# Huangying-Zhan/DF-VO

Hardware: AMD Instinct MI355X
Metric: KITTI-odom frames/sec (DF-VO per-pair tracking hot path: monodepth2 + LiteFlowNet fwd/bwd + kp selection + E/H RANSAC + scale) (higher is better)
Workload: dtype f32 (f16x3 split products: two f16 planes per operand = 22 mantissa bits, three exact products per term, fp32 accumulate; direct one- / two-channel heads exact fp32)

## Files before the change

df-vo_amd/csrc/conv_taps_f16s.hip:

```cpp
#include "dfvo_common.h"


namespace dfvo {

#include "conv_epi.h"
#include "conv_f16_split.h"

typedef unsigned int u32x4t __attribute__((ext_vector_type(4)));
typedef unsigned int u32x2t __attribute__((ext_vector_type(2)));
typedef __attribute__((address_space(4))) const u32x4t cu32x4t;

template <int TH, int TC, int NP = 3, int PF = 3>
__global__ __launch_bounds__(64 * TH) void conv_taps_f16s_kernel(const ConvParams p, int G, int pxd, int wcols, int wrows) {
    extern __shared__ __attribute__((aligned(16))) unsigned char taps_lds[];
    constexpr int NT = 64 * TH;
    const int t = threadIdx.x, lane = t & 63;
    const int wave = __builtin_amdgcn_readfirstlane(t >> 6);
    const int lp = lane & 31, kb = lane >> 5;
    const int tiles_x = (p.Wo + 31) / 32, tiles_y = (p.Ho + TH - 1) / TH;
    const int nb = gridDim.x;
    int bid = blockIdx.x;
    {
        const int q = nb >> 3, r = nb & 7, xcd = bid & 7, k = bid >> 3;
        bid = (xcd < r ? xcd * (q + 1) : r * (q + 1) + (xcd - r) * q) + k;
    }
    const int n = bid / (tiles_y * tiles_x);
    const int trem = bid - n * (tiles_y * tiles_x);
    const int oy0 = (trem / tiles_x) * TH, ox0 = (trem % tiles_x) * 32;
    const int iy0 = oy0 * p.stride - p.pad_h, ix0 = ox0 * p.stride - p.pad_w;

    float amax = 0.f;
    const int npix = wrows * wcols;
    const int zoff = npix * pxd;
    if (t < 4) reinterpret_cast<unsigned*>(taps_lds + zoff)[t] = 0u;
    {
        const int dpx = NT / G, dcg = NT - dpx * G;
        const int dwy = dpx / wcols, dwx = dpx - dwy * wcols;
        int px = t / G, cg = t - px * G;
        int wy = px / wcols, wx = px - wy * wcols;
        constexpr int LB = 4;
        const int nitems = npix * G;
        for (int it = t; it < nitems; it += NT * LB) {
            f32x4 xb[LB];
            int pxb[LB], cgb[LB];
#pragma unroll
            for (int u = 0; u < LB; ++u) {
                const bool live = it + u * NT < nitems;
                const int iy = iy0 + wy, ix = ix0 + wx;
                const bool v = live && iy >= 0 && iy < p.H && ix >= 0 && ix < p.W;
                pxb[u] = live ? px : -1;
                cgb[u] = cg;
                xb[u] = f32x4{0.f, 0.f, 0.f, 0.f};
                if (v) xb[u] = *reinterpret_cast<const f32x4*>(p.src0 + ((size_t)(n * p.H + iy) * p.W + ix) * p.cs0 + p.co0 + cg * 4);
                cg += dcg;
                int cpx = dpx;
                if (cg >= G) {
                    cg -= G;
                    cpx += 1;
                }
                px += cpx;
                wx += dwx + (cpx - dpx);
                wy += dwy;
                if (wx >= wcols) {
                    wx -= wcols;
                    wy += 1;
                }
                if (wx >= wcols) {
                    wx -= wcols;
                    wy += 1;
                }
            }
#pragma unroll
            for (int u = 0; u < LB; ++u) {
                if (pxb[u] < 0) continue;
                h16x4 hi, lo;
                unsigned char* d = taps_lds + (size_t)pxb[u] * pxd + cgb[u] * 8;
                if constexpr (NP == 3) {
                    split_f16_planes(xb[u], &hi, &lo, amax);
                    *reinterpret_cast<h16x4*>(d) = hi;
                    *reinterpret_cast<h16x4*>(d + G * 8) = lo;
                } else {
                    split_f16_hi(xb[u], &hi, amax);
                    *reinterpret_cast<h16x4*>(d) = hi;
                }
            }
        }
    }
    const int S = p.f16g_steps;
    const int rowb = wcols * pxd, lo_off = G * 8;
    int* const otab = reinterpret_cast<int*>(taps_lds + zoff + 16);
    for (int i = t; i < S * 4; i += NT) {
        const unsigned e = p.f16g_tab[i];
        const int ky = e & 31, kx = (e >> 5) & 31, cg = (int)(e >> 16) >> 2;
        otab[i] = ((e >> 10) & 1u) ? ky * rowb + kx * pxd + cg * 8 : -1;
    }
    __syncthreads();

    const unsigned short* const wbase = p.wf16g + (size_t)(kb * 32 + lp) * 8;
    const size_t w_step_stride = (size_t)p.wf16g_cout_pad * 32;
    const int lane_base = (wave * p.stride * wcols + lp * p.stride) * pxd;

    h16x8 rw[PF][TC][2];
    u32x2t rx[PF][2][2];
    int nl = 0;
    u32x2t oo = *reinterpret_cast<const u32x2t*>(otab + 2 * kb);
    auto load_step = [&](int st) {
        const int o0 = (int)oo[0], o1 = (int)oo[1];
        oo = *reinterpret_cast<const u32x2t*>(otab + (nl + 1 < S ? nl + 1 : S - 1) * 4 + 2 * kb);
#pragma unroll
        for (int j = 0; j < 2; ++j) {
            const int o = j ? o1 : o0;
            const int a_hi = o < 0 ? zoff : lane_base + o;
            const int a_lo = o < 0 ? zoff + 8 : lane_base + o + lo_off;
            rx[st][j][0] = *reinterpret_cast<const u32x2t*>(taps_lds + a_hi);
            if constexpr (NP == 3) rx[st][j][1] = *reinterpret_cast<const u32x2t*>(taps_lds + a_lo);
        }
        const unsigned short* g = wbase + (size_t)nl * w_step_stride;
#pragma unroll
        for (int i = 0; i < TC; ++i) {
            rw[st][i][0] = *reinterpret_cast<const h16x8*>(g + (size_t)i * 1024);
            if constexpr (NP == 3) rw[st][i][1] = *reinterpret_cast<const h16x8*>(g + (size_t)i * 1024 + 512);
        }
        ++nl;
    };
    f32x16 am[TC], ax[TC];
#pragma unroll
    for (int i = 0; i < TC; ++i)
#pragma unroll
        for (int e = 0; e < 16; ++e) am[i][e] = ax[i][e] = 0.f;
#pragma unroll
    for (int d = 0; d < PF; ++d)
        if (d < S) load_step(d);
    for (int s = 0; s < S; s += PF) {
#pragma unroll
        for (int u = 0; u < PF; ++u) {
            if (s + u < S) {
                const u32x4t hq = {rx[u][0][0][0], rx[u][0][0][1], rx[u][1][0][0], rx[u][1][0][1]};
                u32x4t lq = {0u, 0u, 0u, 0u};
                if constexpr (NP == 3) lq = u32x4t{rx[u][0][1][0], rx[u][0][1][1], rx[u][1][1][0], rx[u][1][1][1]};
                const h16x8 xh = __builtin_bit_cast(h16x8, hq), xl = __builtin_bit_cast(h16x8, lq);
                h16x8 wh[TC], wl[TC];
#pragma unroll
                for (int i = 0; i < TC; ++i) {
                    wh[i] = rw[u][i][0];
                    if constexpr (NP == 3) wl[i] = rw[u][i][1];
                }
                if (s + u + PF < S) load_step(u);
                if constexpr (NP == 3) {
#pragma unroll
                    for (int i = 0; i < TC; ++i) ax[i] = __builtin_amdgcn_mfma_f32_32x32x16_f16(wh[i], xl, ax[i], 0, 0, 0);
#pragma unroll
                    for (int i = 0; i < TC; ++i) ax[i] = __builtin_amdgcn_mfma_f32_32x32x16_f16(wl[i], xh, ax[i], 0, 0, 0);
                }
#pragma unroll
                for (int i = 0; i < TC; ++i) am[i] = __builtin_amdgcn_mfma_f32_32x32x16_f16(wh[i], xh, am[i], 0, 0, 0);
            }
        }
    }
    if (amax > F16S_MAX) atomicAdd(p.f16s_clamp_ctr, 1u);

    const int oy = oy0 + wave, ox = ox0 + lp;
    if (oy >= p.Ho || ox >= p.Wo) return;
    float* const drow = p.dst + (((size_t)n * p.Ho + oy) * p.Wo + ox) * p.dst_cs + p.dst_co;
    const float slope = p.act == ACT_LEAKY ? p.act_param : 1.f;
    f32x4 bq[4 * TC];
#pragma unroll
    for (int q = 0; q < 4 * TC; ++q) {
        const int col0 = (q >> 2) * 32 + 8 * (q & 3) + 4 * kb;
        bq[q] = *reinterpret_cast<const f32x4*>(p.bias + (col0 + 3 < p.cout_pad ? col0 : p.cout_pad - 4));
    }
#pragma unroll
    for (int q = 0; q < 4 * TC; ++q) {
        const int col0 = (q >> 2) * 32 + 8 * (q & 3) + 4 * kb;
        f32x4 x;
#pragma unroll
        for (int e = 0; e < 4; ++e) {
            const float v = am[q >> 2][4 * (q & 3) + e] + F16S_LO_UNSCALE * ax[q >> 2][4 * (q & 3) + e] + bq[q][e];
            x[e] = (v > 0.f || v != v) ? v : (p.act == ACT_RELU ? 0.f : v * slope);
        }
        if (col0 + 3 < p.cout) {
            *reinterpret_cast<f32x4*>(drow + col0) = x;
        } else {
#pragma unroll
            for (int e = 0; e < 4; ++e) {
                if (col0 + e < p.cout)
                    drow[col0 + e] = x[e];
                else if (col0 + e < p.dst_zero_to)
                    drow[col0 + e] = 0.f;
            }
        }
    }
}

namespace {
struct TapsGeom {
    int G, pxd, th, wrows, wcols;
    size_t lds;
};
bool taps_geom(const ConvParams& p, TapsGeom* g) {
    g->G = p.G0;
    g->pxd = p.G0 * 16 + 8;
    for (int th = 4; th >= 2; th -= 2) {
        g->th = th;
        g->wrows = (th - 1) * p.stride + p.kh;
        g->wcols = 31 * p.stride + p.kw;
        g->lds = (size_t)g->wrows * g->wcols * g->pxd + 16 + (size_t)p.f16g_steps * 16;
        if (g->lds <= 48 * 1024) return true;
    }
    return false;
}
template <int TH, int TC>
void taps_launch(const ConvParams& p, hipStream_t stream, int tiles, const TapsGeom& g) {
    with_f16_terms(p, [&](auto np) {
        hipLaunchKernelGGL((conv_taps_f16s_kernel<TH, TC, decltype(np)::value>), dim3(tiles), dim3(64 * TH), g.lds, stream, p, g.G,
                           g.pxd, g.wcols, g.wrows);
    });
}
}

bool conv_taps_f16s_ok(const ConvParams& p) {
    if (!p.wf16g || !p.f16g_tab || p.G1 != 0 || p.up0 != 0 || p.pad_mode != PAD_ZERO) return false;
    if (p.kh * p.kw < 3 || p.stride != 1 || p.kh > 31 || p.kw > 31) return false;
    if (p.wf16g_cout_pad != 32 && p.wf16g_cout_pad != 64) return false;
    if ((p.cs0 | p.co0) & 3) return false;
    if (p.res || ((p.dst_cs | p.dst_co) & 3) || p.cout_pad < 4 || (p.act != ACT_NONE && p.act != ACT_LEAKY && p.act != ACT_RELU)) return false;
    TapsGeom g;
    return taps_geom(p, &g);
}

int launch_taps_f16s(const ConvParams& p, hipStream_t stream) {
    DFVO_ARG_CHECK(p.f16s_clamp_ctr, "conv_taps_f16s: clamp counter not set");
    TapsGeom g;
    DFVO_ARG_CHECK(taps_geom(p, &g), "conv_taps_f16s: window does not fit");
    const int tiles = p.N * ((p.Ho + g.th - 1) / g.th) * ((p.Wo + 31) / 32);
    const bool tc2 = p.wf16g_cout_pad == 64;
    ConvProfScope prof(p, stream, 20);
    if (g.th == 4)
        tc2 ? taps_launch<4, 2>(p, stream, tiles, g) : taps_launch<4, 1>(p, stream, tiles, g);
    else
        tc2 ? taps_launch<2, 2>(p, stream, tiles, g) : taps_launch<2, 1>(p, stream, tiles, g);
    DFVO_HIP_CHECK(hipGetLastError());
    return prof.done(tiles, 0, 7);
}

}
```

Before: 321.5.

## Stage conv weights in LDS with taller tiles for 7-wide stride-1 taps convs

Adds a weight-in-LDS variant of the f16-split taps convolution. Each block copies all filter steps into dynamic shared memory (up to 160KB) and uses taller output tiles (8 or 16 rows) for stride-1 convs with a 7-tap kernel dimension. The goal is to cut repeated global/L2 weight fetches per tile and amortise the input window over more output rows. It also adds an env-gated stride-2 path that uses a deinterleaved even/odd column layout. The trade is heavy LDS use per block, which lowers occupancy, plus a smaller prefetch depth for the tall tiles.

```diff
diff --git a/df-vo_amd/csrc/conv_taps_f16s.hip b/df-vo_amd/csrc/conv_taps_f16s.hip
--- a/df-vo_amd/csrc/conv_taps_f16s.hip
+++ b/df-vo_amd/csrc/conv_taps_f16s.hip
@@ -10,8 +10,8 @@
 typedef unsigned int u32x2t __attribute__((ext_vector_type(2)));
 typedef __attribute__((address_space(4))) const u32x4t cu32x4t;
 
-template <int TH, int TC, int NP = 3, int PF = 3>
-__global__ __launch_bounds__(64 * TH) void conv_taps_f16s_kernel(const ConvParams p, int G, int pxd, int wcols, int wrows) {
+template <int TH, int TC, int NP = 3, int PF = 3, bool WL = false>
+__global__ __launch_bounds__(64 * TH) void conv_taps_f16s_kernel(const ConvParams p, int G, int pxd, int wcols, int wrows, int half) {
     extern __shared__ __attribute__((aligned(16))) unsigned char taps_lds[];
     constexpr int NT = 64 * TH;
     const int t = threadIdx.x, lane = t & 63;
@@ -48,7 +48,7 @@
                 const bool live = it + u * NT < nitems;
                 const int iy = iy0 + wy, ix = ix0 + wx;
                 const bool v = live && iy >= 0 && iy < p.H && ix >= 0 && ix < p.W;
-                pxb[u] = live ? px : -1;
+                pxb[u] = !live ? -1 : half ? wy * wcols + (wx & 1) * half + (wx >> 1) : px;
                 cgb[u] = cg;
                 xb[u] = f32x4{0.f, 0.f, 0.f, 0.f};
                 if (v) xb[u] = *reinterpret_cast<const f32x4*>(p.src0 + ((size_t)(n * p.H + iy) * p.W + ix) * p.cs0 + p.co0 + cg * 4);
@@ -92,13 +92,30 @@
     for (int i = t; i < S * 4; i += NT) {
         const unsigned e = p.f16g_tab[i];
         const int ky = e & 31, kx = (e >> 5) & 31, cg = (int)(e >> 16) >> 2;
-        otab[i] = ((e >> 10) & 1u) ? ky * rowb + kx * pxd + cg * 8 : -1;
+        const int kc = half ? (kx & 1) * half + (kx >> 1) : kx;
+        otab[i] = ((e >> 10) & 1u) ? ky * rowb + kc * pxd + cg * 8 : -1;
+    }
+    const int woff = (zoff + 16 + S * 16 + 15) & ~15;
+    if constexpr (WL) {
+        const u32x4t* const wsrc = reinterpret_cast<const u32x4t*>(p.wf16g);
+        u32x4t* const wdst = reinterpret_cast<u32x4t*>(taps_lds + woff);
+        const int nw = S * TC * 128;
+        for (int i = t; i < nw; i += NT * 4) {
+            u32x4t wv[4];
+#pragma unroll
+            for (int u = 0; u < 4; ++u)
+                if (i + u * NT < nw) wv[u] = wsrc[i + u * NT];
+#pragma unroll
+            for (int u = 0; u < 4; ++u)
+                if (i + u * NT < nw) wdst[i + u * NT] = wv[u];
+        }
     }
     __syncthreads();
 
     const unsigned short* const wbase = p.wf16g + (size_t)(kb * 32 + lp) * 8;
     const size_t w_step_stride = (size_t)p.wf16g_cout_pad * 32;
-    const int lane_base = (wave * p.stride * wcols + lp * p.stride) * pxd;
+    const int lane_base = (wave * p.stride * wcols + (half ? lp : lp * p.stride)) * pxd;
+    const unsigned char* const wlds = taps_lds + woff + lane * 16;
 
     h16x8 rw[PF][TC][2];
     u32x2t rx[PF][2][2];
@@ -115,11 +132,20 @@
             rx[st][j][0] = *reinterpret_cast<const u32x2t*>(taps_lds + a_hi);
             if constexpr (NP == 3) rx[st][j][1] = *reinterpret_cast<const u32x2t*>(taps_lds + a_lo);
         }
-        const unsigned short* g = wbase + (size_t)nl * w_step_stride;
-#pragma unroll
-        for (int i = 0; i < TC; ++i) {
-            rw[st][i][0] = *reinterpret_cast<const h16x8*>(g + (size_t)i * 1024);
-            if constexpr (NP == 3) rw[st][i][1] = *reinterpret_cast<const h16x8*>(g + (size_t)i * 1024 + 512);
+        if constexpr (WL) {
+            const unsigned char* g = wlds + nl * (TC * 2048);
+#pragma unroll
+            for (int i = 0; i < TC; ++i) {
+                rw[st][i][0] = *reinterpret_cast<const h16x8*>(g + i * 2048);
+                if constexpr (NP == 3) rw[st][i][1] = *reinterpret_cast<const h16x8*>(g + i * 2048 + 1024);
+            }
+        } else {
+            const unsigned short* g = wbase + (size_t)nl * w_step_stride;
+#pragma unroll
+            for (int i = 0; i < TC; ++i) {
+                rw[st][i][0] = *reinterpret_cast<const h16x8*>(g + (size_t)i * 1024);
+                if constexpr (NP == 3) rw[st][i][1] = *reinterpret_cast<const h16x8*>(g + (size_t)i * 1024 + 512);
+            }
         }
         ++nl;
     };
@@ -194,33 +220,68 @@
 
 namespace {
 struct TapsGeom {
-    int G, pxd, th, wrows, wcols;
+    int G, pxd, th, wrows, wcols, half;
+    bool wl;
     size_t lds;
 };
+constexpr size_t TAPS_LDS_STATIC = 48 * 1024;
+constexpr size_t TAPS_LDS_MAX = 160 * 1024;
+
+int taps_forced_th() {
+    static const int th = [] {
+        const char* v = getenv("DFVO_TAPS_TH");
+        const int x = v ? atoi(v) : 0;
+        return x == 4 || x == 8 || x == 16 ? x : 0;
+    }();
+    return th;
+}
+
+bool taps_fit(const ConvParams& p, int th, bool wl, TapsGeom* g) {
+    g->th = th;
+    g->wl = wl;
+    g->wrows = (th - 1) * p.stride + p.kh;
+    const size_t win = (size_t)g->wrows * g->wcols * g->pxd + 16 + (size_t)p.f16g_steps * 16;
+    g->lds = wl ? (win + 15) / 16 * 16 + (size_t)p.f16g_steps * p.wf16g_cout_pad * 64 : win;
+    return g->lds <= (wl ? TAPS_LDS_MAX : TAPS_LDS_STATIC);
+}
+
 bool taps_geom(const ConvParams& p, TapsGeom* g) {
     g->G = p.G0;
     g->pxd = p.G0 * 16 + 8;
-    for (int th = 4; th >= 2; th -= 2) {
-        g->th = th;
-        g->wrows = (th - 1) * p.stride + p.kh;
-        g->wcols = 31 * p.stride + p.kw;
-        g->lds = (size_t)g->wrows * g->wcols * g->pxd + 16 + (size_t)p.f16g_steps * 16;
-        if (g->lds <= 48 * 1024) return true;
-    }
+    g->wcols = 31 * p.stride + p.kw;
+    g->half = p.stride == 2 ? (g->wcols + 1) / 2 : 0;
+    if (const int th = taps_forced_th()) {
+        if (taps_fit(p, th, true, g)) return true;
+    } else if (p.stride == 1 && (p.kh == 7 || p.kw == 7)) {
+        for (int th = p.kw == 1 ? 16 : 8; th >= 8; th >>= 1) {
+            const long long tiles = (long long)p.N * ((p.Ho + th - 1) / th) * ((p.Wo + 31) / 32);
+            if (p.Ho >= 2 * th && tiles >= 256 && taps_fit(p, th, true, g)) return true;
+        }
+    }
+    for (int th = 4; th >= 2; th -= 2)
+        if (taps_fit(p, th, false, g)) return true;
     return false;
 }
-template <int TH, int TC>
-void taps_launch(const ConvParams& p, hipStream_t stream, int tiles, const TapsGeom& g) {
-    with_f16_terms(p, [&](auto np) {
-        hipLaunchKernelGGL((conv_taps_f16s_kernel<TH, TC, decltype(np)::value>), dim3(tiles), dim3(64 * TH), g.lds, stream, p, g.G,
-                           g.pxd, g.wcols, g.wrows);
+template <int TH, int TC, bool WL>
+int taps_launch(const ConvParams& p, hipStream_t stream, int tiles, const TapsGeom& g) {
+    return with_f16_terms(p, [&](auto np) -> int {
+        const auto kernel = conv_taps_f16s_kernel<TH, TC, decltype(np)::value, WL ? (TH == 16 ? 1 : 2) : 3, WL>;
+        if (g.lds > TAPS_LDS_STATIC)
+            if (int rc_lds = ensure_dyn_lds((const void*)kernel, g.lds)) return rc_lds;
+        hipLaunchKernelGGL(kernel, dim3(tiles), dim3(64 * TH), g.lds, stream, p, g.G, g.pxd, g.wcols, g.wrows, g.half);
+        return DFVO_OK;
     });
+}
+template <int TH, bool WL>
+int taps_launch_tc(const ConvParams& p, hipStream_t stream, int tiles, const TapsGeom& g) {
+    return p.wf16g_cout_pad == 64 ? taps_launch<TH, 2, WL>(p, stream, tiles, g) : taps_launch<TH, 1, WL>(p, stream, tiles, g);
 }
 }
 
 bool conv_taps_f16s_ok(const ConvParams& p) {
     if (!p.wf16g || !p.f16g_tab || p.G1 != 0 || p.up0 != 0 || p.pad_mode != PAD_ZERO) return false;
-    if (p.kh * p.kw < 3 || p.stride != 1 || p.kh > 31 || p.kw > 31) return false;
+    if (p.kh * p.kw < 3 || p.kh > 31 || p.kw > 31) return false;
+    if (p.stride != 1 && !(p.stride == 2 && taps_forced_th())) return false;
     if (p.wf16g_cout_pad != 32 && p.wf16g_cout_pad != 64) return false;
     if ((p.cs0 | p.co0) & 3) return false;
     if (p.res || ((p.dst_cs | p.dst_co) & 3) || p.cout_pad < 4 || (p.act != ACT_NONE && p.act != ACT_LEAKY && p.act != ACT_RELU)) return false;
@@ -233,14 +294,16 @@
     TapsGeom g;
     DFVO_ARG_CHECK(taps_geom(p, &g), "conv_taps_f16s: window does not fit");
     const int tiles = p.N * ((p.Ho + g.th - 1) / g.th) * ((p.Wo + 31) / 32);
-    const bool tc2 = p.wf16g_cout_pad == 64;
     ConvProfScope prof(p, stream, 20);
-    if (g.th == 4)
-        tc2 ? taps_launch<4, 2>(p, stream, tiles, g) : taps_launch<4, 1>(p, stream, tiles, g);
+    int rc;
+    if (!g.wl)
+        rc = g.th == 4 ? taps_launch_tc<4, false>(p, stream, tiles, g) : taps_launch_tc<2, false>(p, stream, tiles, g);
     else
-        tc2 ? taps_launch<2, 2>(p, stream, tiles, g) : taps_launch<2, 1>(p, stream, tiles, g);
+        rc = g.th == 16 ? taps_launch_tc<16, true>(p, stream, tiles, g)
+                        : g.th == 8 ? taps_launch_tc<8, true>(p, stream, tiles, g) : taps_launch_tc<4, true>(p, stream, tiles, g);
+    if (rc != DFVO_OK) return rc;
     DFVO_HIP_CHECK(hipGetLastError());
-    return prof.done(tiles, 0, 7);
-}
-
-}
+    return prof.done(tiles, g.wl ? g.th : 0, 7);
+}
+
+}
```

Measured after the change: 322.9 (median of 6 runs). No clear change (+0.4%).
